# lh3/minimap2

Hardware: AMD Instinct MI355X
Metric: aligned Gbases/sec (map-ont, 10 kb reads, -a) (higher is better)
Workload: dtype int8 (ksw2 difference DP) / int32+f32 (chaining)

## Files before the change

minimap2_amd/__init__.py:

```python
import ctypes as C
import os

_HERE = os.path.dirname(os.path.abspath(__file__))
LIB_PATH = os.path.join(_HERE, "libmm2amd.so")


class Mm2AmdError(RuntimeError):
    pass


class KswJob(C.Structure):
    _fields_ = [("query", C.c_void_p), ("target", C.c_void_p), ("qlen", C.c_int32), ("tlen", C.c_int32), ("w", C.c_int32),
                ("zdrop", C.c_int32), ("end_bonus", C.c_int32), ("flag", C.c_int32)]


class FinJob(C.Structure):
    _fields_ = [("query", C.c_void_p), ("target", C.c_void_p), ("qlen", C.c_int32), ("tlen", C.c_int32), ("n_pieces", C.c_int32),
                ("piece", C.POINTER(C.POINTER(C.c_uint32))), ("piece_len", C.POINTER(C.c_int32))]


class FinRes(C.Structure):
    _fields_ = [("n_cigar", C.c_int32), ("blen", C.c_int32), ("mlen", C.c_int32), ("n_ambi", C.c_int32), ("dp_max", C.c_int32), ("qshift", C.c_int32),
                ("tshift", C.c_int32), ("is_spliced", C.c_int32), ("cigar_off", C.c_uint32)]

# ... 1197 lines not shown
        rc = lib().mm2amd_idx_getseq(self._idx, rid, start, end, buf)
        if rc < 0:
            _check(rc)
        return buf.raw.translate(_CODE_TO_BASE).decode("ascii")

    def map_pairs(self, pairs, text=False, cs=False, MD=False, ds=False):
        self.stage(pairs)
        if not text:
            return self.run(cs=cs, MD=MD, ds=ds)
        n_reg, reg, rep_len = self.run(raw=True)
        try:
            return self.format_raw(n_reg, reg, rep_len)
        finally:
            self.free_raw(n_reg, reg)

    def last_stats(self):
        v = (C.c_double * 48)()
        k = lib().mm2amd_last_stats(v, 48)
        names = ["t_seed_chain", "t_host_pre", "t_plan", "t_ksw", "t_consume", "t_finish", "n_jobs", "n_rounds", "dp_cells", "dev_allocs", "pin_allocs",
                 "alloc_ns", "cpu_seed_chain", "cpu_host_pre", "cpu_plan", "cpu_ksw", "cpu_consume", "cpu_finish", "n_long_join_dev", "n_long_join_host",
                 "drv_cpu_seed_chain", "drv_cpu_host_pre", "drv_cpu_plan", "drv_cpu_ksw", "drv_cpu_consume", "drv_cpu_finish", "n_early_sub",
                 "n_region_reads_dev", "n_region_reads_host", "n_band128", "n_band256", "n_band_widened", "n_band_rectangle",
                 "arena_dev_bytes", "arena_pin_bytes", "arena_dev_used", "arena_pin_used", "n_band512", "n_band_rectangle_big",
                 "n_anchors_prune_in", "n_anchors_prune_kept", "n_reads_prune_redo"]
        return dict(zip(names, list(v)[:k]))


class SplitWriter(object):

    def __init__(self, prefix, aligner, part_no):
        self._al, self._h = aligner, None
        self._h = lib().mm2amd_split_open(os.fsencode(prefix), aligner._idx, part_no)
        if not self._h:
            _check(lib().mm2amd_last_error_code())

    def write(self, n_seq, n_reg, reg, rep_len, frag_gap):
        _check(lib().mm2amd_split_write(self._h, C.byref(self._al.map_opt), n_seq, n_reg, reg, rep_len, frag_gap))

    def close(self):
        if self._h:
            h, self._h = self._h, None
            _check(lib().mm2amd_split_close(h))

    def __del__(self):
        try:
            self.close()
        except Exception:
# ... 140 lines not shown
```

minimap2_amd/csrc/backend_hip.cpp:

```cpp
#include <atomic>
#include <condition_variable>
#include <algorithm>
#include <cstdio>
#include <cstring>
#include <memory>
#include <mutex>
#include <numeric>
#include <stdexcept>
#include <thread>
#include "backend.hpp"
#include "chain_dump.hpp"
#include "chain_host.hpp"
#include "device_ctx.hpp"
#include "ksw_host.hpp"
#include "seed_chain_dev.hpp"
#include "index_build.hpp"
#include "kernel_prof.hpp"
#include "threads.hpp"
#include "trace.hpp"
#include "sdust_core.hpp"
#include "sdust.hpp"

namespace mm2amd {

extern const uint8_t kNt4Table[256];

namespace {

bool env_on(const char *name) { const char *e = getenv(name); return e && *e && strcmp(e, "0") != 0; }

struct Lane {
	int id = 0;
	int set = 0;
	hipStream_t stream = nullptr;
	SeedChainBuffers B{};
	KswRunner ksw;
	DevBuf<uint64_t> d_a_off, d_mp_off, d_mz_x, d_mz_y, d_minipos, d_skey_in, d_sval_in, d_skey_out, d_sval_out;
	DevBuf<uint32_t> d_sdust_list;
	DevBuf<SdustCounters> d_sdust_cnt;
	PinBuf<SdustCounters> h_sdust_cnt;
	DevBuf<uint32_t> d_mz_cnt, d_sd_n, d_sd_off, d_sd_aoff, d_sd_qpos, d_sd_info, d_n_anchor, d_n_minipos, d_n_seedhit, d_tie, d_nkept;
	DevBuf<int32_t> d_rep_len, d_f, d_p, d_t;
	DevBuf<Anchor> d_anchors;
	DevBuf<uint8_t> d_tbytes;
	DevBuf<uint32_t> d_sort_list;
	PinBuf<uint32_t> h_sort_list;
	DevBuf<Anchor> d_dump_anchors;
	DevBuf<uint32_t> d_pieces;
	PinBuf<uint32_t> h_pieces, h_lj_pieces;
	DevBuf<Anchor> d_lj_out_a;
	DevBuf<uint64_t> d_lj_src;
	PinBuf<Anchor> h_lj_a;
	PinBuf<uint64_t> h_lj_u, h_lj_off, h_lj_aoff, h_lj_uoff;
	PinBuf<int32_t> h_lj_nu, h_lj_nv;
	PinBuf<uint32_t> h_lj_tie, h_lj_list;
	PinBuf<unsigned long long> h_lj_cursor;
	DevBuf<FinRegion> d_fin_regions; DevBuf<FinPiece> d_fin_pieces; DevBuf<uint32_t> d_fin_out; DevBuf<FinResult> d_fin_res;
	PinBuf<FinRegion> h_fin_regions; PinBuf<FinPiece> h_fin_pieces; PinBuf<uint32_t> h_fin_out; PinBuf<FinResult> h_fin_res;
	struct EqxBufs { DevBuf<uint32_t> d_n, d_out; DevBuf<uint64_t> d_off; PinBuf<uint32_t> h_n, h_out; PinBuf<uint64_t> h_off; };
	EqxBufs eqx_fin, eqx_rg;
	long rg_lo = 0; size_t rg_n = 0; uint64_t rg_n_v = 0, rg_n_v2 = 0, rg_n_u = 0, rg_n_u2 = 0;
	std::vector<int8_t> rg_src; std::vector<uint64_t> rg_aoff, rg_uoff; std::vector<int32_t> rg_nu, rg_nv;
	DevBuf<uint64_t> d_lj_out_u;
// ... 124 lines not shown
			memcpy(h + seq_off_[i], reads[i].seq, reads[i].len);
			if (reads[i].paired()) memcpy(h + seq_off_[i] + reads[i].len, reads[i].seq2, reads[i].len2);
		}, 64);
		d_qpool_.ensure(2 * total + 16);
		d_seq_off_.ensure(n + 1);
		n_units_ = n;
		if (has_pairs_) {
			unit_first_.resize(n + 1);
			unit_first_[0] = 0;
			for (size_t i = 0; i < n; ++i) unit_first_[i + 1] = unit_first_[i] + (reads[i].paired() ? 2 : 1);
			n_units_ = (size_t)unit_first_[n];
			unit_off_.resize(n_units_ + 1);
			for (size_t i = 0; i < n; ++i) {
				unit_off_[unit_first_[i]] = seq_off_[i];
				if (reads[i].paired()) unit_off_[unit_first_[i] + 1] = seq_off_[i] + (uint64_t)reads[i].len;
			}
			unit_off_[n_units_] = total;
			d_unit_off_.ensure(n_units_ + 1), d_unit_first_.ensure(n + 1);
			HIP_CHECK(hipMemcpyAsync(d_unit_off_.p, unit_off_.data(), (n_units_ + 1) * 8, hipMemcpyHostToDevice, stream_));
			HIP_CHECK(hipMemcpyAsync(d_unit_first_.p, unit_first_.data(), (n + 1) * 4, hipMemcpyHostToDevice, stream_));
		}
		HIP_CHECK(hipMemcpyAsync(d_seq_off_.p, seq_off_.data(), (n + 1) * 8, hipMemcpyHostToDevice, stream_));
		read_names_.clear();
		if (getenv("MM2AMD_SEED_DUMP") || chain_dump_path()) for (size_t i = 0; i < n; ++i) read_names_.push_back(reads[i].name);
		have_read_names_ = false;
		if (name_rules_ && n > 0) {
			have_read_names_ = true;
			for (size_t i = 0; i < n; ++i) if (!reads[i].name) { have_read_names_ = false; break; }
		}
		if (have_read_names_) {
			name_key_.resize(2 * n);
			parallel_for_side(n_threads_, (long)n, [&](long i, int) {
				const std::string q(reads[i].name);
				const size_t lb = (size_t)(std::lower_bound(sorted_names_.begin(), sorted_names_.end(), q) - sorted_names_.begin());
				name_key_[i] = (int32_t)lb;
				name_key_[n + i] = lb < sorted_names_.size() && sorted_names_[lb] == q ? (int32_t)lb : -1;
			}, 256);
			d_name_key_.ensure(2 * n);
			HIP_CHECK(hipMemcpyAsync(d_name_key_.p, name_key_.data(), 2 * n * 4, hipMemcpyHostToDevice, stream_));
		}
		stream_wait(stream_);
	}
	void activate_batch() override { cur_ = 1 - cur_; }
	int current_set() const override { return cur_; }
	void bind_lane(int lane, int set) override { lanes_.at(lane)->set = set; }
	bool stages_beside_mapping() const override { return true; }

// ... 19 lines not shown
		B = SeedChainBuffers();
		B.n_reads = (int)n, B.seq_off = d_seq_off_.p + lo, B.ascii = h_ascii_.p, B.qpool = d_qpool_.p;
		if (have_read_names_) B.name_lb = d_name_key_.p + lo, B.name_eq = d_name_key_.p + seq_off_.size() - 1 + lo;
		KernelProfiler &kp = kernel_profiler(lane_id, replica_);
		double tt = Trace::now();
		const double L = (double)(seq_off_[hi] - seq_off_[lo]);
		SeedChainBuffers Bu = B;
		const size_t ulo = has_pairs_ ? (size_t)unit_first_[lo] : (size_t)lo, n_unit = has_pairs_ ? (size_t)unit_first_[hi] - ulo : n;
		if (has_pairs_) Bu.n_reads = (int)n_unit, Bu.seq_off = d_unit_off_.p + ulo;
		kp.begin(st); launch_encode(Bu, st); kp.end(st, "encode_kernel", 3 * L);
		const uint64_t base0 = seq_off_[lo], cap_mz = seq_off_[hi] - base0;
		ln.d_mz_cnt.ensure(n_unit);
		ln.d_mz_x.ensure(cap_mz + 1), ln.d_mz_y.ensure(cap_mz + 1);
		ln.d_sd_n.ensure(cap_mz + 1), ln.d_sd_off.ensure(cap_mz + 1), ln.d_sd_aoff.ensure(cap_mz + 1), ln.d_sd_qpos.ensure(cap_mz + 1), ln.d_sd_info.ensure(cap_mz + 1);
		B.mz_cnt = ln.d_mz_cnt.p, B.mz_off = B.seq_off, B.mz_x = ln.d_mz_x.p - base0, B.mz_y = ln.d_mz_y.p - base0;
		B.sd_n = ln.d_sd_n.p - base0, B.sd_off = ln.d_sd_off.p - base0, B.sd_aoff = ln.d_sd_aoff.p - base0, B.sd_qpos = ln.d_sd_qpos.p - base0, B.sd_info = ln.d_sd_info.p - base0;
		const double est_mz = 2.0 * L / (P.w + 1);
		Bu.mz_cnt = B.mz_cnt, Bu.mz_off = Bu.seq_off, Bu.mz_x = B.mz_x, Bu.mz_y = B.mz_y;
		int max_len = 0;
		for (size_t u = 0; u < n_unit; ++u) {
			const uint64_t l_u = has_pairs_ ? unit_off_[ulo + u + 1] - unit_off_[ulo + u] : seq_off_[lo + u + 1] - seq_off_[lo + u];
			max_len = (int)std::max<uint64_t>((uint64_t)max_len, l_u);
		}
		kp.begin(st); launch_sketch(Bu, P, max_len, st); kp.end(st, "sketch_kernel", L + 16.0 * est_mz);
		if (has_pairs_)
			B.unit_first = d_unit_first_.p + lo, B.unit_off = d_unit_off_.p, B.unit_cnt = ln.d_mz_cnt.p - ulo, B.mz_cnt = nullptr;
		const bool dev_sdust = P.sdust_thres > 0 && env_on("MM2AMD_DEVICE_SDUST"), sdust_no_narrow = env_on("MM2AMD_SDUST_NO_NARROW");
		if (dev_sdust) {
			ln.d_sdust_list.ensure(n_unit), ln.d_sdust_cnt.ensure(1);
			HIP_CHECK(hipMemsetAsync(ln.d_sdust_cnt.p, 0, sizeof(SdustCounters), st));
			SdustParams S;
			S.codes = B.qpool, S.off = Bu.seq_off, S.code_mul = 2, S.n_reads = (int)n_unit, S.T = P.sdust_thres < kSdustMaxT ? P.sdust_thres : kSdustMaxT;
			S.reg_n = B.sd_n, S.reg_s = B.sd_off, S.reg_e = B.sd_aoff, S.wide_list = ln.d_sdust_list.p, S.cnt = ln.d_sdust_cnt.p;
			const char *e_cap = getenv("MM2AMD_SDUST_NARROW_CAP");
			const long cap = e_cap && *e_cap ? strtol(e_cap, nullptr, 10) : kSdustNarrowCap;
			if (sdust_no_narrow) {
				S.cap = kSdustWideCap, S.wide = 2;
				kp.begin(st); sdust_launch(S, 0, st); kp.end(st, "sdust_kernel[wide]", 0.0);
			} else {
				S.cap = (int)(cap < 1 ? 1 : cap > kSdustWideCap ? kSdustWideCap : cap), S.wide = 0;
				kp.begin(st); sdust_launch(S, 0, st); kp.end(st, "sdust_kernel[narrow]", 0.0);
				S.cap = kSdustWideCap, S.wide = 1;
				kp.begin(st); sdust_launch(S, 0, st); kp.end(st, "sdust_kernel[wide]", 0.0);
			}
			HIP_CHECK(hipMemcpyAsync(ln.h_sdust_cnt.ensure(1), ln.d_sdust_cnt.p, sizeof(SdustCounters), hipMemcpyDeviceToHost, st));
			kp.begin(st); launch_dust_filter(B, st); kp.end(st, "dust_filter_kernel", 16.0 * est_mz);
		} else if (P.sdust_thres > 0) {
// ... 6 lines not shown
				thread_local std::vector<uint8_t> codes;
				codes.resize((size_t)len + 1);
				for (int j = 0; j < len; ++j) codes[j] = kNt4Table[(uint8_t)asc[o + j]];
				SdustState S;
				S.P = perf.data();
				uint32_t k = 0;
				sdust_scan(codes.data(), len, P.sdust_thres, S, [&](int s0, int e0) { h_s[o - base0 + k] = (uint32_t)s0, h_e[o - base0 + k] = (uint32_t)e0; ++k; });
				if (len > 0) h_n[o - base0] = k;
			}, 16);
			HIP_CHECK(hipMemcpyAsync(ln.d_sd_n.p, h_n, cap_mz * 4, hipMemcpyHostToDevice, st));
			HIP_CHECK(hipMemcpyAsync(ln.d_sd_off.p, h_s, cap_mz * 4, hipMemcpyHostToDevice, st));
			HIP_CHECK(hipMemcpyAsync(ln.d_sd_aoff.p, h_e, cap_mz * 4, hipMemcpyHostToDevice, st));
			kp.begin(st); launch_dust_filter(B, st); kp.end(st, "dust_filter_kernel", 16.0 * est_mz);
		}
		ln.d_n_anchor.ensure(n), ln.d_n_minipos.ensure(n), ln.d_n_seedhit.ensure(n), ln.d_rep_len.ensure(n);
		B.n_anchor = ln.d_n_anchor.p, B.n_minipos = ln.d_n_minipos.p, B.n_seedhit = ln.d_n_seedhit.p, B.rep_len = ln.d_rep_len.p;
		kp.begin(st); launch_seed_collect(B, I_, P, st); kp.end(st, "seed_collect_kernel", 36.0 * est_mz);
		uint32_t *h_na = ln.h_na.ensure(n), *h_nmp = ln.h_nmp.ensure(n);
		int32_t *h_rep = ln.h_rep.ensure(n);
		HIP_CHECK(hipMemcpyAsync(h_na, ln.d_n_anchor.p, n * 4, hipMemcpyDeviceToHost, st));
		HIP_CHECK(hipMemcpyAsync(h_nmp, ln.d_n_minipos.p, n * 4, hipMemcpyDeviceToHost, st));
		HIP_CHECK(hipMemcpyAsync(h_rep, ln.d_rep_len.p, n * 4, hipMemcpyDeviceToHost, st));
		stream_wait(st);
		if (dev_sdust) {
			const SdustCounters &c = *ln.h_sdust_cnt.p;
			if (c.err) throw HipError("[mm2amd] sdust_kernel: a list of perfect intervals outgrew the wide capacity");
			kp.add_units("sdust_kernel[wide]", (double)c.wide_bases);
			if (!sdust_no_narrow) kp.add_units("sdust_kernel[narrow]", L - (double)c.wide_bases + (double)c.narrow_partial);
		}
		Trace::get().add(lane_id, "gpu:sketch+collect", tt, Trace::now()); tt = Trace::now();
		std::vector<uint64_t> &a_off = ln.a_off, &mp_off = ln.mp_off;
		a_off.resize(n + 1), mp_off.resize(n + 1);
		a_off[0] = mp_off[0] = 0;
		for (size_t i = 0; i < n; ++i) a_off[i + 1] = a_off[i] + h_na[i], mp_off[i + 1] = mp_off[i] + h_nmp[i];
		const uint64_t n_a = a_off[n], n_mp = mp_off[n];
		uint64_t *h_off = ln.h_off.ensure(2 * (n + 1));
		memcpy(h_off, a_off.data(), (n + 1) * 8), memcpy(h_off + n + 1, mp_off.data(), (n + 1) * 8);
		ln.d_a_off.ensure(n + 1), ln.d_mp_off.ensure(n + 1);
		HIP_CHECK(hipMemcpyAsync(ln.d_a_off.p, h_off, (n + 1) * 8, hipMemcpyHostToDevice, st));
		HIP_CHECK(hipMemcpyAsync(ln.d_mp_off.p, h_off + n + 1, (n + 1) * 8, hipMemcpyHostToDevice, st));
		ln.d_anchors.ensure(n_a + 1), ln.d_minipos.ensure(n_mp + 1), ln.d_f.ensure(n_a + 1), ln.d_p.ensure(n_a + 1), ln.d_t.ensure(n_a + 1);
		ln.d_skey_in.ensure(n_a + 1), ln.d_sval_in.ensure(n_a + 1), ln.d_skey_out.ensure(n_a + 1), ln.d_sval_out.ensure(n_a + 1), ln.d_tie.ensure(2 * n + 1);
		B.sort_key_in = ln.d_skey_in.p, B.sort_val_in = ln.d_sval_in.p, B.sort_key_out = ln.d_skey_out.p, B.sort_val_out = ln.d_sval_out.p, B.tie_flag = ln.d_tie.p;
		B.tie_list = ln.d_tie.p + n, B.tie_count = ln.d_tie.p + 2 * n;
		B.rid_bits = rid_bits_;
		static const bool prune_env = !(getenv("MM2AMD_ANCHOR_PRUNE") && atoi(getenv("MM2AMD_ANCHOR_PRUNE")) == 0);
// ... 787 lines not shown
```

minimap2_amd/csrc/capi_kernels.cpp:

```cpp
#include <mutex>
#include <string>
#include <vector>
#include <cstring>
#include "../../include/mm2amd.h"
#include "hip_util.hpp"
#include "device_ctx.hpp"
#include "ksw_host.hpp"
#include "kernel_prof.hpp"
#include "region_finish.hpp"
#include "cigar_eqx.hpp"
#include "aln_text.hpp"
#include "junc_text.hpp"
#include "ksw_ll.hpp"
#include "sdust.hpp"
#include "sdust_core.hpp"
#include "hits_merge.hpp"
#include "split_merge.hpp"
#include "index_handle.hpp"
#include "fastx.hpp"
#include "threads.hpp"
#include "trace.hpp"
#include "device_sort.hpp"
#include "seed_chain_dev.hpp"
#include <map>
// ... 1087 lines not shown
			if (l) memcpy(h + o, seqs[i], l);
			o += l;
		}
		d_pool.ensure(2 * total + 32, 1.0), d_off.ensure(n_units + 1, 1.0);
		HIP_CHECK(hipMemsetAsync(d_pool.p, 0xff, 2 * total + 32, dc.stream));
		HIP_CHECK(hipMemcpyAsync(d_off.p, unit_off.data(), (n_units + 1) * 8, hipMemcpyHostToDevice, dc.stream));
		SeedChainBuffers B;
		B.n_reads = (int)(frag_unit[hi] - frag_unit[lo]), B.seq_off = d_off.p + frag_unit[lo], B.ascii = h, B.qpool = d_pool.p + 16;
		launch_encode(B, dc.stream);
		HIP_CHECK(hipMemcpyAsync(out, d_pool.p, 2 * total + 32, hipMemcpyDeviceToHost, dc.stream));
		HIP_CHECK(hipStreamSynchronize(dc.stream));
		return 0;
	});
}

long long mm2amd_alloc_counter(int which)
{
	AllocStats &a = alloc_stats();
	BandCounters &b = band_counters();
	return which == 0 ? a.dev_allocs.load() : which == 1 ? a.pin_allocs.load() : which == 2 ? a.ns.load() : which == 3 ? (long long)b.n_band1.load() : which == 4 ? (long long)b.n_band2.load() :
	       which == 5 ? (long long)b.n_widened.load() : which == 6 ? (long long)b.n_retried.load() :
	       which == 7 ? (long long)dev_arena().held_bytes() : which == 8 ? (long long)pin_arena().held_bytes() : which == 9 ? (long long)dev_arena().used_bytes() : which == 10 ? (long long)pin_arena().used_bytes() :
	       which == 11 ? (long long)b.n_band4.load() : which == 12 ? (long long)b.n_retried_big.load() :
	       which == 13 ? (long long)prune_counters().n_in.load() : which == 14 ? (long long)prune_counters().n_kept.load() : (long long)prune_counters().n_redo.load();
}

void mm2amd_profile_enable(int on)
{
	for (int r = 0; r < kMaxReplicas; ++r) for (int l = 0; l < kMaxProfLanes; ++l) kernel_profiler(l, r).reset();
	KernelProfiler::enabled_flag() = on != 0;
}

int mm2amd_profile_get(mm2amd_kernel_stat_t *out, int cap)
{
	std::map<std::string, KernelStat> all;
	for (int r = 0; r < kMaxReplicas; ++r) for (int l = 0; l < kMaxProfLanes; ++l)
		for (const auto &kv : kernel_profiler(l, r).stats()) {
			KernelStat &k = all[kv.first];
			k.ms += kv.second.ms, k.alg_bytes += kv.second.alg_bytes, k.units += kv.second.units, k.launches += kv.second.launches;
		}
	int n = 0;
	for (const auto &kv : all) {
		if (n >= cap) break;
		mm2amd_kernel_stat_t &o = out[n++];
		memset(&o, 0, sizeof o);
		strncpy(o.name, kv.first.c_str(), sizeof o.name - 1);
		o.ms = kv.second.ms, o.alg_bytes = kv.second.alg_bytes, o.launches = kv.second.launches, o.units = kv.second.units;
// ... 6 lines not shown
```

minimap2_amd/csrc/capi_map.cpp:

```cpp
#include <algorithm>
#include <condition_variable>
#include <cstdlib>
#include <cstring>
#include <memory>
#include <atomic>
#include <mutex>
#include <shared_mutex>
#include <string>
#include <thread>
#include "../../include/mm2amd.h"
#include "mapper.hpp"
#include "format.hpp"
#include "index_handle.hpp"
#include "threads.hpp"

namespace mm2amd {
int effective_cpus();
Backend *make_backend(const FlatIndex &fi, void *device_tables, int n_threads, int device, int replica, int tables_device);
int backend_device_count();
void *backend_build_index_tables(FlatIndex &fi, int device, int *on_device);
void backend_free_index_tables(void *tables);
const char *backend_name();
void capi_set_error(const std::string &msg);
int capi_fail(int code, const std::string &msg);
// ... 668 lines not shown
	std::unique_lock<std::shared_mutex> lk(g_ctx_mu);
	if (!g_ctx || g_ctx->generation != generation) return 0;
	g_ctx.reset();
	return 1;
}

const char *mm2amd_backend_name(void) { return backend_name(); }
int mm2amd_format_fraction(double v, char *buf) { return buf ? format_fraction_for_test(v, buf) : 0; }

int mm2amd_last_stats(double *v, int n)
{
	std::shared_lock<std::shared_mutex> lk(g_ctx_mu);
	if (!g_ctx) return 0;
	std::lock_guard<std::mutex> lk_stats(g_ctx->stats_mu);
	const MapperStats &s = g_ctx->stats;
	const double a[] = { s.t_seed_chain, s.t_host_pre, s.t_plan, s.t_ksw, s.t_consume, s.t_finish, (double)s.n_jobs, (double)s.n_rounds, s.dp_cells,
	                     (double)mm2amd_alloc_counter(0), (double)mm2amd_alloc_counter(1), (double)mm2amd_alloc_counter(2),
	                     s.c_seed_chain, s.c_host_pre, s.c_plan, s.c_ksw, s.c_consume, s.c_finish, (double)s.n_long_join_dev, (double)s.n_long_join_host,
	                     s.d_seed_chain, s.d_host_pre, s.d_plan, s.d_ksw, s.d_consume, s.d_finish, (double)s.n_early_sub,
	                     (double)s.n_region_reads_dev, (double)s.n_region_reads_host,
	                     (double)mm2amd_alloc_counter(3), (double)mm2amd_alloc_counter(4), (double)mm2amd_alloc_counter(5), (double)mm2amd_alloc_counter(6),
	                     (double)mm2amd_alloc_counter(7), (double)mm2amd_alloc_counter(8), (double)mm2amd_alloc_counter(9), (double)mm2amd_alloc_counter(10),
	                     (double)mm2amd_alloc_counter(11), (double)mm2amd_alloc_counter(12),
	                     (double)mm2amd_alloc_counter(13), (double)mm2amd_alloc_counter(14), (double)mm2amd_alloc_counter(15) };
	int k = 0;
	for (; k < n && k < (int)(sizeof a / sizeof a[0]); ++k) v[k] = a[k];
	return k;
}

}
```

minimap2_amd/csrc/hip_util.hpp:

```cpp
#pragma once
#include <hip/hip_runtime.h>
#include <time.h>
#include <cstdio>
#include <cstdlib>
#include <cstdint>
#include <stdexcept>
#include <string>
#include <atomic>
#include <chrono>
#include <map>
#include <mutex>
#include <vector>
#include <iterator>

#ifdef MM2AMD_WAVE_EMU
#define MM2_DYN_LDS(T, name) T *const name = (T *)wave_emu::dyn_shared()
#define MM2_LOCKSTEP() __builtin_amdgcn_wave_barrier()
#else
#define MM2_DYN_LDS(T, name) extern __shared__ __attribute__((aligned(16))) T name[]
#define MM2_LOCKSTEP() ((void)0)
#endif

namespace mm2amd {

// ... 27 lines not shown
	}
	HIP_CHECK(hipEventRecord(slot->ev, s));
	static const long max_ns = [] { const char *e = getenv("MM2AMD_WAIT_MAX_US"); const long us = e ? atol(e) : 500; return (us < 20 ? 20 : us) * 1000L; }();
	long ns = 20000;
	for (int it = 0;; ++it) {
		const hipError_t e = hipEventQuery(slot->ev);
		if (e == hipSuccess) return;
		if (e != hipErrorNotReady) HIP_CHECK(e);
		if (it < 4) continue;
		timespec ts = { 0, ns };
		nanosleep(&ts, nullptr);
		if (ns < max_ns) ns += ns / 2;
	}
}

int effective_cpus();

struct AllocStats { std::atomic<long> dev_allocs{0}, pin_allocs{0}; std::atomic<double> dummy{0}; std::atomic<long long> dev_bytes{0}, pin_bytes{0}; std::atomic<long long> ns{0}; };
inline AllocStats &alloc_stats() { static AllocStats s; return s; }
struct BandCounters { std::atomic<unsigned long long> n_band1{0}, n_band2{0}, n_band4{0}, n_widened{0}, n_retried{0}, n_retried_big{0}; };
inline BandCounters &band_counters() { static BandCounters s; return s; }
struct PruneCounters { std::atomic<unsigned long long> n_in{0}, n_kept{0}, n_redo{0}; };
inline PruneCounters &prune_counters() { static PruneCounters s; return s; }

class MemArena {
public:
	MemArena(bool pinned, size_t chunk_bytes) : pinned_(pinned), chunk_bytes_(chunk_bytes) {}
	~MemArena() { for (Chunk &c : chunks_) raw_free(c.base); for (auto &kv : solo_) raw_free(kv.first); }
	static bool enabled()
	{
#ifdef MM2AMD_WAVE_EMU
		static const bool on = getenv("MM2AMD_ARENA") != nullptr;
#else
		static const bool on = getenv("MM2AMD_NO_ARENA") == nullptr;
#endif
		return on;
	}
	void *alloc(size_t bytes)
	{
		bytes = (bytes + 255) & ~(size_t)255;
		if (bytes == 0) bytes = 256;
		int dev = 0;
		(void)hipGetDevice(&dev);
		if (!enabled() || bytes > chunk_bytes_ / 2) {
			char *p = raw_alloc(bytes);
			std::lock_guard<std::mutex> lk(mu_);
// ... 129 lines not shown
```

minimap2_amd/csrc/seed_chain.hip:

```cpp
#include <hip/hip_runtime.h>
#include "hip_util.hpp"
#include "seed_chain_dev.hpp"
#include "index_build.hpp"
#include "heap_order.hpp"
#include "sdust_core.hpp"
#include "sketch_dev.hpp"
#include "sdust_dev.hpp"
#include "kernel_prof.hpp"

namespace mm2amd {

#define WAVE_SYNC() do { __builtin_amdgcn_fence(__ATOMIC_ACQ_REL, "wavefront"); __builtin_amdgcn_wave_barrier(); } while (0)

__constant__ uint8_t c_nt4[256];
extern const uint8_t kNt4Table[256];
static bool g_nt4_uploaded = false;

static void upload_tables(hipStream_t s)
{
	if (g_nt4_uploaded) return;
	HIP_CHECK(hipMemcpyToSymbolAsync(HIP_SYMBOL(c_nt4), kNt4Table, 256, 0, hipMemcpyHostToDevice, s));
	g_nt4_uploaded = true;
}

constexpr int kEncodeBlocks = 64, kEncodeDepth = 4;

__device__ __forceinline__ int encode_owner(const uint64_t *seq_off, int lo, int n, uint64_t p)
{
	int step = 1;
// ... 129 lines not shown
	}
	if (min_x != UINT64_MAX) EMIT_MZ(min_x, min_y);
#undef EMIT_MZ
	B.mz_cnt[r] = n_out;
}

__device__ __forceinline__ uint32_t wave_prefix_add_u32(uint32_t v);
struct SketchLds {
	int ring_bytes, pk_words, tile_cap, per_wave;
};
__host__ __device__ inline SketchLds sketch_lds_layout(int w, int tile_cap)
{
	SketchLds L;
	L.tile_cap = tile_cap;
	L.ring_bytes = 64 * w * 12;
	if (L.ring_bytes < 1024) L.ring_bytes = 1024;
	L.pk_words = (tile_cap + 256) / 16;
	L.per_wave = L.ring_bytes + (L.pk_words + 2) * 4 + L.pk_words * 2 + tile_cap / 8;
	L.per_wave = (L.per_wave + 15) & ~15;
	return L;
}
constexpr int SK_WARM_LDS = 128, SK_TAIL_LDS = 128;

template <bool K32, int W>
__global__ void __launch_bounds__(64) sketch_wave_kernel(SeedChainBuffers B, int w, int k, int tile_cap)
{
	MM2_DYN_LDS(uint64_t, lds);
	const int lane = threadIdx.x;
	const int r = blockIdx.x;
	const SketchLds L = sketch_lds_layout(w, tile_cap);
	uint64_t *const bx = lds + lane;
	uint32_t *const by = (uint32_t *)(lds + (size_t)w * 64) + lane;
	uint32_t *const pk = (uint32_t *)((uint8_t *)lds + L.ring_bytes) + 2;
	uint16_t *const amb = (uint16_t *)(pk + L.pk_words);
	uint32_t *const marks = (uint32_t *)(amb + L.pk_words);
	uint16_t *const list = (uint16_t *)lds;
	const int list_cap = L.ring_bytes / 2;
	const uint64_t o = B.seq_off[r];
	const int64_t len = (int64_t)(B.seq_off[r + 1] - o);
	const uint8_t *seq = B.qpool + 2 * o;
	uint64_t *const ox = B.mz_x + B.mz_off[r], *const oy = B.mz_y + B.mz_off[r];
	if (lane == 0) pk[-1] = pk[-2] = 0;
	const int64_t n_tiles = len > tile_cap ? (len + tile_cap - 1) / tile_cap : 1;
	const int64_t tile = n_tiles > 1 ? ((len + n_tiles - 1) / n_tiles + 63) & ~(int64_t)63 : len;
	uint32_t n_out = 0;
	for (int64_t t0 = 0; t0 < len; t0 += tile) {
		const int64_t t1 = t0 + tile < len ? t0 + tile : len;
		const int64_t lo = t0 >= SK_WARM_LDS ? t0 - SK_WARM_LDS : 0;
		const int64_t hi = t1 + SK_TAIL_LDS < len ? t1 + SK_TAIL_LDS : len;
		for (int64_t c = lo + 16 * lane; c < hi; c += 16 * 64) {
			struct __attribute__((packed, aligned(1))) Q16 { uint32_t v[4]; };
			const Q16 q = *(const Q16 *)(seq + c);
			const uint32_t qv[4] = { q.v[0], q.v[1], q.v[2], q.v[3] };
			uint32_t packed, flags;
			sk_pack16(qv, &packed, &flags);
			pk[(c - lo) >> 4] = packed, amb[(c - lo) >> 4] = (uint16_t)flags;
		}
		for (int64_t i = lane; i < (t1 - t0 + 31) >> 5; i += 64) marks[i] = 0;
		WAVE_SYNC();
		int64_t chunk = (t1 - t0 + 63) / 64;
		if (chunk < 32) chunk = 32;
		const int64_t cs = t0 + (int64_t)lane * chunk, ce = cs + chunk < t1 ? cs + chunk : t1;
		if (cs < t1) {
			uint32_t wpk = 0, wamb = 0;
			int64_t wcur = -1;
			auto base_at = [&](int64_t i) -> int {
				if (i >= lo && i < hi) {
					const int64_t rel = i - lo;
					if ((rel >> 4) != wcur) wcur = rel >> 4, wpk = pk[wcur], wamb = amb[wcur];
					return (wamb >> (rel & 15) & 1u) ? 4 : (int)(wpk >> (30 - 2 * (int)(rel & 15)) & 3u);
				}
				return (int)seq[i];
			};
			sketch_chunk_core<false, K32, uint32_t, W>(base_at, len, cs, ce, w, k, 0u, bx, by, 64, [&](uint64_t, uint64_t y) {
				const uint32_t rel = (uint32_t)((int64_t)((uint32_t)y >> 1) - t0);
				atomicOr(&marks[rel >> 5], 1u << (rel & 31));
			}, (int64_t)(w + k + 8));
		}
		WAVE_SYNC();
		const int n_words = (int)((t1 - t0 + 31) >> 5);
		int words_per_round = list_cap / 32;
		if (words_per_round > 64) words_per_round = 64;
		for (int w0 = 0; w0 < n_words; w0 += words_per_round) {
			uint32_t m = lane < words_per_round && w0 + lane < n_words ? marks[w0 + lane] : 0u;
			const uint32_t cnt = (uint32_t)__popc(m);
			const uint32_t incl = wave_prefix_add_u32(cnt);
			const uint32_t total = (uint32_t)__builtin_amdgcn_readlane((int32_t)incl, 63);
			uint32_t at = incl - cnt;
			while (m) {
				list[at++] = (uint16_t)(((w0 + lane) << 5) + __builtin_ctz(m));
				m &= m - 1;
			}
			WAVE_SYNC();
			for (uint32_t e = lane; e < total; e += 64) {
				const int64_t pos = t0 + (int64_t)list[e];
				uint64_t x, y;
				sk_minimizer_at(pk, pos - lo, pos, k, &x, &y);
				ox[n_out + e] = x, oy[n_out + e] = y;
			}
			n_out += total;
			WAVE_SYNC();
		}
	}
	if (lane == 0) B.mz_cnt[r] = n_out;
}

void launch_sketch(const SeedChainBuffers &B, const SeedChainParams &P, int max_len, void *stream)
{
	hipStream_t s = (hipStream_t)stream;
	if (!P.is_hpc && P.w <= 32) {
		int tile_cap = (std::max(max_len, 1024) + 1023) & ~1023;
		if (tile_cap > 16384) tile_cap = 16384;
		static const int force_tile = getenv("MM2AMD_SKETCH_TILE") ? atoi(getenv("MM2AMD_SKETCH_TILE")) : 0;
		if (force_tile >= 64) tile_cap = force_tile & ~63;
		const SketchLds L = sketch_lds_layout(P.w, tile_cap);
#define MM2_SKETCH_LAUNCH(K32_, W_) hipLaunchKernelGGL((sketch_wave_kernel<K32_, W_>), dim3(B.n_reads), dim3(64), (size_t)L.per_wave, s, B, P.w, P.k, tile_cap)
		static const bool generic_only = getenv("MM2AMD_SKETCH_GENERIC") != nullptr;
		const bool k32 = 2 * P.k <= 32;
		if (generic_only) { if (k32) MM2_SKETCH_LAUNCH(true, 0); else MM2_SKETCH_LAUNCH(false, 0); }
		else if (k32 && P.w == 10) MM2_SKETCH_LAUNCH(true, 10);
		else if (k32 && P.w == 5) MM2_SKETCH_LAUNCH(true, 5);
		else if (!k32 && P.w == 19) MM2_SKETCH_LAUNCH(false, 19);
		else if (!k32 && P.w == 10) MM2_SKETCH_LAUNCH(false, 10);
		else if (k32) MM2_SKETCH_LAUNCH(true, 0);
		else MM2_SKETCH_LAUNCH(false, 0);
#undef MM2_SKETCH_LAUNCH
	} else {
		const dim3 grid((B.n_reads + 63) / 64), block(64);
		if (P.w <= 32) hipLaunchKernelGGL((sketch_kernel<32>), grid, block, 0, s, B, P.w, P.k, P.is_hpc);
		else hipLaunchKernelGGL((sketch_kernel<256>), grid, block, 0, s, B, P.w, P.k, P.is_hpc);
	}
	HIP_CHECK(hipGetLastError());
}

__global__ void __launch_bounds__(64) dust_filter_kernel(SeedChainBuffers B)
{
	const int r = blockIdx.x * 64 + threadIdx.x;
	if (r >= B.n_reads) return;
	const int32_t u0 = B.unit_first ? B.unit_first[r] : 0, nu = B.unit_first ? B.unit_first[r + 1] - u0 : 1;
	for (int32_t k = 0; k < nu; ++k) {
		const uint64_t o = B.unit_first ? B.unit_off[u0 + k] : B.seq_off[r];
		uint32_t *cnt = B.unit_first ? const_cast<uint32_t *>(B.unit_cnt) + (u0 + k) : B.mz_cnt + r;
		const uint32_t *rs = B.sd_off + o, *re = B.sd_aoff + o;
		const int n_reg = (int)B.sd_n[o];
		if (n_reg == 0) continue;
		const int pos_off = B.unit_first ? (int)(o - B.unit_off[u0]) : 0;
		*cnt = (uint32_t)dust_filter_minimizers((int)*cnt, B.mz_x + o, B.mz_y + o, n_reg,
			[&](int u, int32_t *st, int32_t *en) { *st = (int32_t)rs[u], *en = (int32_t)re[u]; }, pos_off);
	}
}

void launch_dust_filter(const SeedChainBuffers &B, void *stream)
{
	hipLaunchKernelGGL(dust_filter_kernel, dim3((B.n_reads + 63) / 64), dim3(64), 0, (hipStream_t)stream, B);
	HIP_CHECK(hipGetLastError());
// ... 1950 lines not shown
```

minimap2_amd/csrc/seed_chain_dev.hpp:

```cpp
#pragma once
#include <cstdint>
#include <cstddef>
#include "types.hpp"
#include "backend.hpp"

namespace mm2amd {

struct DevIndex {
	const uint32_t *bucket_start;
	const uint64_t *keys;
	const uint32_t *val_off;
	const struct IdxSlot *slots;
	const struct IdxSlot *first;
	const uint64_t *pos;
	const uint32_t *S;
	int bucket_bits, key_shift;
	const int32_t *name_rank;
	const uint32_t *seq_len;
};

struct SeedChainBuffers {
	int n_reads;
	const uint64_t *seq_off;
	const char *ascii;
	uint8_t *qpool;
	const int32_t *name_lb, *name_eq;
	const int32_t *unit_first;
	const uint64_t *unit_off;
	const uint32_t *unit_cnt;
	uint32_t *mz_cnt;
	const uint64_t *mz_off;
	uint64_t *mz_x, *mz_y;
	uint32_t *sd_n, *sd_off, *sd_aoff, *sd_qpos, *sd_info;
	uint32_t *n_anchor, *n_minipos, *n_seedhit;
	int32_t *rep_len;
	const uint64_t *a_off;
	const uint64_t *mp_off;
	Anchor *anchors;
	uint64_t *sort_key_in, *sort_val_in;
	uint64_t *sort_key_out, *sort_val_out;
	uint32_t *tie_flag;
	uint32_t *tie_list, *tie_count;
	int rid_bits;
	uint32_t *n_kept = nullptr;
	uint32_t *redo_list = nullptr, *redo_count = nullptr;
	int prune_bins = 0, prune_cap = 0;
	uint64_t *mini_pos;
	int32_t *f, *p, *t;
	const uint32_t *pieces = nullptr;
	int n_pieces = 0, piece_len = 0;
	int rmq_rank_max = 256;
	int piece_dense = 0;
	unsigned long long *bt_cursor;
	Anchor *bt_out_a;
	uint64_t *bt_out_u;
// ... 22 lines not shown
```

Baseline: 3.806.

## Add windowed parallel minimizer sketch with dirty-block sequential fallback

Adds a sketch kernel variant in which each lane of the wave evaluates one position, computing its hash key in parallel into an LDS ring. Each position is then tested directly for being a window minimizer by comparing it with its W neighbours. Only 64-position blocks that contain ties, ambiguous bases or nearby edges are recomputed with the existing sequential per-chunk core. This is intended to replace the mostly serial per-lane chunk scan, and its duplicated warm-up work, with data-parallel evaluation. It becomes the default for common w/k pairs and adds block/dirty counters, a per-call device-to-host copy, and extra LDS usage that could reduce occupancy.

```diff
diff --git a/minimap2_amd/__init__.py b/minimap2_amd/__init__.py
--- a/minimap2_amd/__init__.py
+++ b/minimap2_amd/__init__.py
@@ -1243,7 +1243,8 @@
                  "drv_cpu_seed_chain", "drv_cpu_host_pre", "drv_cpu_plan", "drv_cpu_ksw", "drv_cpu_consume", "drv_cpu_finish", "n_early_sub",
                  "n_region_reads_dev", "n_region_reads_host", "n_band128", "n_band256", "n_band_widened", "n_band_rectangle",
                  "arena_dev_bytes", "arena_pin_bytes", "arena_dev_used", "arena_pin_used", "n_band512", "n_band_rectangle_big",
-                 "n_anchors_prune_in", "n_anchors_prune_kept", "n_reads_prune_redo"]
+                 "n_anchors_prune_in", "n_anchors_prune_kept", "n_reads_prune_redo",
+                 "n_sketch_blocks", "n_sketch_blocks_dirty"]
         return dict(zip(names, list(v)[:k]))
 
 
diff --git a/minimap2_amd/csrc/backend_hip.cpp b/minimap2_amd/csrc/backend_hip.cpp
--- a/minimap2_amd/csrc/backend_hip.cpp
+++ b/minimap2_amd/csrc/backend_hip.cpp
@@ -39,6 +39,8 @@
 	DevBuf<uint32_t> d_sdust_list;
 	DevBuf<SdustCounters> d_sdust_cnt;
 	PinBuf<SdustCounters> h_sdust_cnt;
+	DevBuf<unsigned long long> d_sk_count; PinBuf<unsigned long long> h_sk_count; unsigned long long sk_seen[2] = { 0, 0 };
+	DevBuf<uint32_t> d_sk_blocks; PinBuf<uint32_t> h_sk_blocks;
 	DevBuf<uint32_t> d_mz_cnt, d_sd_n, d_sd_off, d_sd_aoff, d_sd_qpos, d_sd_info, d_n_anchor, d_n_minipos, d_n_seedhit, d_tie, d_nkept;
 	DevBuf<int32_t> d_rep_len, d_f, d_p, d_t;
 	DevBuf<Anchor> d_anchors;
@@ -209,7 +211,7 @@
 		}
 		HIP_CHECK(hipMemcpyAsync(d_seq_off_.p, seq_off_.data(), (n + 1) * 8, hipMemcpyHostToDevice, stream_));
 		read_names_.clear();
-		if (getenv("MM2AMD_SEED_DUMP") || chain_dump_path()) for (size_t i = 0; i < n; ++i) read_names_.push_back(reads[i].name);
+		if (getenv("MM2AMD_SEED_DUMP") || getenv("MM2AMD_SKETCH_TRACE") || chain_dump_path()) for (size_t i = 0; i < n; ++i) read_names_.push_back(reads[i].name);
 		have_read_names_ = false;
 		if (name_rules_ && n > 0) {
 			have_read_names_ = true;
@@ -275,7 +277,15 @@
 			const uint64_t l_u = has_pairs_ ? unit_off_[ulo + u + 1] - unit_off_[ulo + u] : seq_off_[lo + u + 1] - seq_off_[lo + u];
 			max_len = (int)std::max<uint64_t>((uint64_t)max_len, l_u);
 		}
+		static const bool sk_trace = getenv("MM2AMD_SKETCH_TRACE") != nullptr;
+		if (!ln.d_sk_count.p) { ln.d_sk_count.ensure(2); HIP_CHECK(hipMemsetAsync(ln.d_sk_count.p, 0, 16, st)); }
+		Bu.sk_count = ln.d_sk_count.p;
+		if (sk_trace) Bu.sk_blocks = ln.d_sk_blocks.ensure(2 * n_unit);
 		kp.begin(st); launch_sketch(Bu, P, max_len, st); kp.end(st, "sketch_kernel", L + 16.0 * est_mz);
+		unsigned long long *h_skc = ln.h_sk_count.ensure(2);
+		HIP_CHECK(hipMemcpyAsync(h_skc, ln.d_sk_count.p, 16, hipMemcpyDeviceToHost, st));
+		uint32_t *h_skb = sk_trace ? ln.h_sk_blocks.ensure(2 * n_unit) : nullptr;
+		if (sk_trace) HIP_CHECK(hipMemcpyAsync(h_skb, ln.d_sk_blocks.p, 2 * n_unit * 4, hipMemcpyDeviceToHost, st));
 		if (has_pairs_)
 			B.unit_first = d_unit_first_.p + lo, B.unit_off = d_unit_off_.p, B.unit_cnt = ln.d_mz_cnt.p - ulo, B.mz_cnt = nullptr;
 		const bool dev_sdust = P.sdust_thres > 0 && env_on("MM2AMD_DEVICE_SDUST"), sdust_no_narrow = env_on("MM2AMD_SDUST_NO_NARROW");
@@ -328,6 +338,19 @@
 		HIP_CHECK(hipMemcpyAsync(h_nmp, ln.d_n_minipos.p, n * 4, hipMemcpyDeviceToHost, st));
 		HIP_CHECK(hipMemcpyAsync(h_rep, ln.d_rep_len.p, n * 4, hipMemcpyDeviceToHost, st));
 		stream_wait(st);
+		{
+			sketch_counters().n_blocks += h_skc[0] - ln.sk_seen[0], sketch_counters().n_dirty += h_skc[1] - ln.sk_seen[1];
+			ln.sk_seen[0] = h_skc[0], ln.sk_seen[1] = h_skc[1];
+			if (sk_trace && !has_pairs_) {
+				std::string txt;
+				char buf[64];
+				for (size_t i = 0; i < n; ++i) {
+					txt += "[mm2amd] SKETCH read ", txt += read_names_.empty() || !read_names_[lo + i] ? "*" : read_names_[lo + i];
+					snprintf(buf, sizeof buf, ": blocks %u dirty %u\n", h_skb[2 * i], h_skb[2 * i + 1]), txt += buf;
+				}
+				fputs(txt.c_str(), stderr);
+			}
+		}
 		if (dev_sdust) {
 			const SdustCounters &c = *ln.h_sdust_cnt.p;
 			if (c.err) throw HipError("[mm2amd] sdust_kernel: a list of perfect intervals outgrew the wide capacity");
diff --git a/minimap2_amd/csrc/capi_kernels.cpp b/minimap2_amd/csrc/capi_kernels.cpp
--- a/minimap2_amd/csrc/capi_kernels.cpp
+++ b/minimap2_amd/csrc/capi_kernels.cpp
@@ -1133,7 +1133,8 @@
 	       which == 5 ? (long long)b.n_widened.load() : which == 6 ? (long long)b.n_retried.load() :
 	       which == 7 ? (long long)dev_arena().held_bytes() : which == 8 ? (long long)pin_arena().held_bytes() : which == 9 ? (long long)dev_arena().used_bytes() : which == 10 ? (long long)pin_arena().used_bytes() :
 	       which == 11 ? (long long)b.n_band4.load() : which == 12 ? (long long)b.n_retried_big.load() :
-	       which == 13 ? (long long)prune_counters().n_in.load() : which == 14 ? (long long)prune_counters().n_kept.load() : (long long)prune_counters().n_redo.load();
+	       which == 13 ? (long long)prune_counters().n_in.load() : which == 14 ? (long long)prune_counters().n_kept.load() : which == 15 ? (long long)prune_counters().n_redo.load() :
+	       which == 16 ? (long long)sketch_counters().n_blocks.load() : (long long)sketch_counters().n_dirty.load();
 }
 
 void mm2amd_profile_enable(int on)
diff --git a/minimap2_amd/csrc/capi_map.cpp b/minimap2_amd/csrc/capi_map.cpp
--- a/minimap2_amd/csrc/capi_map.cpp
+++ b/minimap2_amd/csrc/capi_map.cpp
@@ -714,7 +714,8 @@
 	                     (double)mm2amd_alloc_counter(3), (double)mm2amd_alloc_counter(4), (double)mm2amd_alloc_counter(5), (double)mm2amd_alloc_counter(6),
 	                     (double)mm2amd_alloc_counter(7), (double)mm2amd_alloc_counter(8), (double)mm2amd_alloc_counter(9), (double)mm2amd_alloc_counter(10),
 	                     (double)mm2amd_alloc_counter(11), (double)mm2amd_alloc_counter(12),
-	                     (double)mm2amd_alloc_counter(13), (double)mm2amd_alloc_counter(14), (double)mm2amd_alloc_counter(15) };
+	                     (double)mm2amd_alloc_counter(13), (double)mm2amd_alloc_counter(14), (double)mm2amd_alloc_counter(15),
+	                     (double)mm2amd_alloc_counter(16), (double)mm2amd_alloc_counter(17) };
 	int k = 0;
 	for (; k < n && k < (int)(sizeof a / sizeof a[0]); ++k) v[k] = a[k];
 	return k;
diff --git a/minimap2_amd/csrc/hip_util.hpp b/minimap2_amd/csrc/hip_util.hpp
--- a/minimap2_amd/csrc/hip_util.hpp
+++ b/minimap2_amd/csrc/hip_util.hpp
@@ -73,6 +73,8 @@
 inline BandCounters &band_counters() { static BandCounters s; return s; }
 struct PruneCounters { std::atomic<unsigned long long> n_in{0}, n_kept{0}, n_redo{0}; };
 inline PruneCounters &prune_counters() { static PruneCounters s; return s; }
+struct SketchCounters { std::atomic<unsigned long long> n_blocks{0}, n_dirty{0}; };
+inline SketchCounters &sketch_counters() { static SketchCounters s; return s; }
 
 class MemArena {
 public:
diff --git a/minimap2_amd/csrc/seed_chain.hip b/minimap2_amd/csrc/seed_chain.hip
--- a/minimap2_amd/csrc/seed_chain.hip
+++ b/minimap2_amd/csrc/seed_chain.hip
@@ -5,6 +5,7 @@
 #include "heap_order.hpp"
 #include "sdust_core.hpp"
 #include "sketch_dev.hpp"
+#include "sketch_window_dev.hpp"
 #include "sdust_dev.hpp"
 #include "kernel_prof.hpp"
 
@@ -180,20 +181,26 @@
 }
 constexpr int SK_WARM_LDS = 128, SK_TAIL_LDS = 128;
 
-template <bool K32, int W>
+template <bool K32, int W, bool WIN = false>
 __global__ void __launch_bounds__(64) sketch_wave_kernel(SeedChainBuffers B, int w, int k, int tile_cap)
 {
 	MM2_DYN_LDS(uint64_t, lds);
+	typedef typename SkwKeyType<K32>::type KT;
 	const int lane = threadIdx.x;
 	const int r = blockIdx.x;
 	const SketchLds L = sketch_lds_layout(w, tile_cap);
+	const SkwLds LW = skw_lds_layout(w, tile_cap, (int)sizeof(KT));
+	const int ring_lanes = WIN ? skw_dirty_lanes(W, (int)sizeof(KT)) : 64, front_bytes = WIN ? LW.front_bytes : L.ring_bytes;
 	uint64_t *const bx = lds + lane;
-	uint32_t *const by = (uint32_t *)(lds + (size_t)w * 64) + lane;
-	uint32_t *const pk = (uint32_t *)((uint8_t *)lds + L.ring_bytes) + 2;
+	uint32_t *const by = (uint32_t *)(lds + (size_t)w * ring_lanes) + lane;
+	KT *const keys = (KT *)((uint8_t *)lds + LW.key_off);
+	uint16_t *const dlist = (uint16_t *)((uint8_t *)lds + LW.dlist_off);
+	uint32_t *const pk = (uint32_t *)((uint8_t *)lds + front_bytes) + 2;
 	uint16_t *const amb = (uint16_t *)(pk + L.pk_words);
 	uint32_t *const marks = (uint32_t *)(amb + L.pk_words);
 	uint16_t *const list = (uint16_t *)lds;
-	const int list_cap = L.ring_bytes / 2;
+	const int list_cap = front_bytes / 2;
+	uint32_t n_blocks = 0, n_dirty = 0;
 	const uint64_t o = B.seq_off[r];
 	const int64_t len = (int64_t)(B.seq_off[r + 1] - o);
 	const uint8_t *seq = B.qpool + 2 * o;
@@ -214,26 +221,74 @@
 			sk_pack16(qv, &packed, &flags);
 			pk[(c - lo) >> 4] = packed, amb[(c - lo) >> 4] = (uint16_t)flags;
 		}
-		for (int64_t i = lane; i < (t1 - t0 + 31) >> 5; i += 64) marks[i] = 0;
+		if (!WIN) for (int64_t i = lane; i < (t1 - t0 + 31) >> 5; i += 64) marks[i] = 0;
 		WAVE_SYNC();
-		int64_t chunk = (t1 - t0 + 63) / 64;
-		if (chunk < 32) chunk = 32;
-		const int64_t cs = t0 + (int64_t)lane * chunk, ce = cs + chunk < t1 ? cs + chunk : t1;
-		if (cs < t1) {
-			uint32_t wpk = 0, wamb = 0;
-			int64_t wcur = -1;
-			auto base_at = [&](int64_t i) -> int {
-				if (i >= lo && i < hi) {
-					const int64_t rel = i - lo;
-					if ((rel >> 4) != wcur) wcur = rel >> 4, wpk = pk[wcur], wamb = amb[wcur];
-					return (wamb >> (rel & 15) & 1u) ? 4 : (int)(wpk >> (30 - 2 * (int)(rel & 15)) & 3u);
-				}
-				return (int)seq[i];
-			};
-			sketch_chunk_core<false, K32, uint32_t, W>(base_at, len, cs, ce, w, k, 0u, bx, by, 64, [&](uint64_t, uint64_t y) {
-				const uint32_t rel = (uint32_t)((int64_t)((uint32_t)y >> 1) - t0);
-				atomicOr(&marks[rel >> 5], 1u << (rel & 31));
-			}, (int64_t)(w + k + 8));
+		uint32_t wpk = 0, wamb = 0;
+		int64_t wcur = -1;
+		auto base_at = [&](int64_t i) -> int {
+			if (i >= lo && i < hi) {
+				const int64_t rel = i - lo;
+				if ((rel >> 4) != wcur) wcur = rel >> 4, wpk = pk[wcur], wamb = amb[wcur];
+				return (wamb >> (rel & 15) & 1u) ? 4 : (int)(wpk >> (30 - 2 * (int)(rel & 15)) & 3u);
+			}
+			return (int)seq[i];
+		};
+		if constexpr (WIN) {
+			const int nb = (int)((t1 - t0 + 63) >> 6), margin = skw_margin(W, k);
+			const bool tiny = len - (k - 1) < W || t1 - t0 < W;
+			uint64_t bad_a = 0, bad_b = 0, nm_prev = 0;
+			int nd = 0;
+			for (int i = -2; i <= nb + 1; ++i) {
+				const int q = 64 * i + lane, pos = (int)t0 + q;
+				const uint64_t nm = __ballot(skw_is_n(amb, pos, (int)lo, (int)hi));
+				KT key = skw_key_at<K32>(pk, pos, (int)lo, (int)hi, k);
+				if (nm | nm_prev) {
+					if (skw_n_spread(nm_prev, nm, k) >> lane & 1) key = 0;
+				}
+				keys[q & 255] = key, keys[(q & 255) + 256] = key;
+				WAVE_SYNC();
+				uint64_t bad_c = 0;
+				if (i >= 0) {
+					const int b = i - 1, x0 = (64 * b) & 255;
+					bool mark, tie;
+					skw_lane_eval<KT, W>(keys + (x0 ? x0 : 256) + lane, &mark, &tie);
+					bad_c = __ballot(tie) | nm_prev;
+					const uint64_t mk = __ballot(mark && pos - 64 >= (int)t0 && pos - 64 < (int)t1);
+					if (b >= 0 && b < nb && lane < 2) marks[2 * b + lane] = (uint32_t)(mk >> (32 * lane));
+				}
+				if (i >= 2 && (tiny || skw_block_dirty(bad_a, bad_b, bad_c, margin))) {
+					if (lane == 0) dlist[nd] = (uint16_t)(i - 2);
+					++nd;
+				}
+				bad_a = bad_b, bad_b = bad_c, nm_prev = nm;
+			}
+			WAVE_SYNC();
+			n_blocks += (uint32_t)nb, n_dirty += (uint32_t)nd;
+			const int quota = skw_dirty_quota(nd, ring_lanes);
+			if (lane < ring_lanes && lane * quota < nd) {
+				const int e1 = (lane + 1) * quota < nd ? (lane + 1) * quota : nd;
+				for (int e = lane * quota; e < e1;) {
+					int f = e + 1;
+					while (f < e1 && dlist[f] == dlist[f - 1] + 1) ++f;
+					const int b0 = dlist[e], b1 = dlist[f - 1] + 1;
+					for (int b = b0; b < b1; ++b) marks[2 * b] = marks[2 * b + 1] = 0;
+					const int64_t cs = t0 + 64 * (int64_t)b0, ce = t0 + 64 * (int64_t)b1 < t1 ? t0 + 64 * (int64_t)b1 : t1;
+					sketch_chunk_core<false, K32, uint32_t, W>(base_at, len, cs, ce, w, k, 0u, bx, by, ring_lanes, [&](uint64_t, uint64_t y) {
+						const uint32_t rel = (uint32_t)((int64_t)((uint32_t)y >> 1) - t0);
+						marks[rel >> 5] |= 1u << (rel & 31);
+					}, (int64_t)margin);
+					e = f;
+				}
+			}
+		} else {
+			int64_t chunk = (t1 - t0 + 63) / 64;
+			if (chunk < 32) chunk = 32;
+			const int64_t cs = t0 + (int64_t)lane * chunk, ce = cs + chunk < t1 ? cs + chunk : t1;
+			if (cs < t1)
+				sketch_chunk_core<false, K32, uint32_t, W>(base_at, len, cs, ce, w, k, 0u, bx, by, 64, [&](uint64_t, uint64_t y) {
+					const uint32_t rel = (uint32_t)((int64_t)((uint32_t)y >> 1) - t0);
+					atomicOr(&marks[rel >> 5], 1u << (rel & 31));
+				}, (int64_t)(w + k + 8));
 		}
 		WAVE_SYNC();
 		const int n_words = (int)((t1 - t0 + 31) >> 5);
@@ -261,20 +316,39 @@
 		}
 	}
 	if (lane == 0) B.mz_cnt[r] = n_out;
+	if (WIN && lane == 0) {
+		if (B.sk_count) {
+			atomicAdd(&B.sk_count[0], (unsigned long long)n_blocks);
+			if (n_dirty) atomicAdd(&B.sk_count[1], (unsigned long long)n_dirty);
+		}
+		if (B.sk_blocks) B.sk_blocks[2 * r] = n_blocks, B.sk_blocks[2 * r + 1] = n_dirty;
+	}
 }
 
 void launch_sketch(const SeedChainBuffers &B, const SeedChainParams &P, int max_len, void *stream)
 {
 	hipStream_t s = (hipStream_t)stream;
+	bool win = false;
 	if (!P.is_hpc && P.w <= 32) {
 		int tile_cap = (std::max(max_len, 1024) + 1023) & ~1023;
 		if (tile_cap > 16384) tile_cap = 16384;
 		static const int force_tile = getenv("MM2AMD_SKETCH_TILE") ? atoi(getenv("MM2AMD_SKETCH_TILE")) : 0;
 		if (force_tile >= 64) tile_cap = force_tile & ~63;
 		const SketchLds L = sketch_lds_layout(P.w, tile_cap);
+		static const bool window_on = !getenv("MM2AMD_SKETCH_WINDOW") || atoi(getenv("MM2AMD_SKETCH_WINDOW")) != 0;
 #define MM2_SKETCH_LAUNCH(K32_, W_) hipLaunchKernelGGL((sketch_wave_kernel<K32_, W_>), dim3(B.n_reads), dim3(64), (size_t)L.per_wave, s, B, P.w, P.k, tile_cap)
 		static const bool generic_only = getenv("MM2AMD_SKETCH_GENERIC") != nullptr;
 		const bool k32 = 2 * P.k <= 32;
+		win = window_on && !generic_only && skw_supported(P.w, P.k) && (k32 ? P.w == 10 || P.w == 5 : P.w == 19 || P.w == 10);
+		const SkwLds LW = skw_lds_layout(P.w, tile_cap, k32 ? 4 : 8);
+#define MM2_SKETCH_LAUNCH_WIN(K32_, W_) hipLaunchKernelGGL((sketch_wave_kernel<K32_, W_, true>), dim3(B.n_reads), dim3(64), (size_t)LW.per_wave, s, B, P.w, P.k, tile_cap)
+		if (win) {
+			if (k32 && P.w == 10) MM2_SKETCH_LAUNCH_WIN(true, 10);
+			else if (k32) MM2_SKETCH_LAUNCH_WIN(true, 5);
+			else if (P.w == 19) MM2_SKETCH_LAUNCH_WIN(false, 19);
+			else MM2_SKETCH_LAUNCH_WIN(false, 10);
+		} else
+#undef MM2_SKETCH_LAUNCH_WIN
 		if (generic_only) { if (k32) MM2_SKETCH_LAUNCH(true, 0); else MM2_SKETCH_LAUNCH(false, 0); }
 		else if (k32 && P.w == 10) MM2_SKETCH_LAUNCH(true, 10);
 		else if (k32 && P.w == 5) MM2_SKETCH_LAUNCH(true, 5);
@@ -289,6 +363,7 @@
 		else hipLaunchKernelGGL((sketch_kernel<256>), grid, block, 0, s, B, P.w, P.k, P.is_hpc);
 	}
 	HIP_CHECK(hipGetLastError());
+	if (B.sk_blocks && !win) HIP_CHECK(hipMemsetAsync(B.sk_blocks, 0, (size_t)B.n_reads * 8, s));
 }
 
 __global__ void __launch_bounds__(64) dust_filter_kernel(SeedChainBuffers B)
diff --git a/minimap2_amd/csrc/seed_chain_dev.hpp b/minimap2_amd/csrc/seed_chain_dev.hpp
--- a/minimap2_amd/csrc/seed_chain_dev.hpp
+++ b/minimap2_amd/csrc/seed_chain_dev.hpp
@@ -31,6 +31,8 @@
 	uint32_t *mz_cnt;
 	const uint64_t *mz_off;
 	uint64_t *mz_x, *mz_y;
+	unsigned long long *sk_count = nullptr;
+	uint32_t *sk_blocks = nullptr;
 	uint32_t *sd_n, *sd_off, *sd_aoff, *sd_qpos, *sd_info;
 	uint32_t *n_anchor, *n_minipos, *n_seedhit;
 	int32_t *rep_len;
diff --git a/minimap2_amd/csrc/sketch_window_dev.hpp b/minimap2_amd/csrc/sketch_window_dev.hpp
--- /dev/null
+++ b/minimap2_amd/csrc/sketch_window_dev.hpp
@@ -0,0 +1,125 @@
+#pragma once
+#include <hip/hip_runtime.h>
+#include <cstdint>
+#include "sketch_dev.hpp"
+
+namespace mm2amd {
+
+template <bool K32> struct SkwKeyType { typedef uint64_t type; };
+template <> struct SkwKeyType<true> { typedef uint32_t type; };
+
+__host__ __device__ inline int skw_margin(int w, int k) { return w + k + 8; }
+__host__ __device__ inline bool skw_supported(int w, int k) { return (k & 1) && w >= 2 && skw_margin(w, k) <= 63 && skw_margin(w, k) + w <= 65; }
+__host__ __device__ inline int skw_dirty_lanes(int w, int key_bytes) { return 32 * w * 12 + 512 * key_bytes + 1024 <= 64 * w * 12 ? 32 : 16; }
+
+template <bool K32>
+__device__ __forceinline__ typename SkwKeyType<K32>::type skw_key_at(const uint32_t *pk, int pos, int lo, int hi, int k)
+{
+	typedef typename SkwKeyType<K32>::type KT;
+	if (pos < lo + k - 1 || pos >= hi) return 0;
+	const int r = pos - lo, j = r >> 4;
+	if (K32) {
+		const uint32_t mask = (1u << 2 * k) - 1u;
+		const uint32_t k0 = (uint32_t)(((uint64_t)pk[j - 1] << 32 | pk[j]) >> (30 - 2 * (r & 15))) & mask;
+#if defined(__has_builtin) && __has_builtin(__builtin_bitreverse32)
+		uint32_t y = __builtin_bitreverse32(k0);
+		y = (y >> 1 & 0x55555555u) | (y & 0x55555555u) << 1;
+		const uint32_t k1 = (y >> (32 - 2 * k)) ^ mask;
+#else
+		const uint32_t k1 = (uint32_t)sk_revcomp(k0, k);
+#endif
+		return (KT)(mm_hash_t<uint32_t>(k0 < k1 ? k0 : k1, mask) + 1u);
+	}
+	const uint64_t mask = (1ULL << 2 * k) - 1ULL;
+	const uint64_t k0 = sk_kmer_at(pk, r, k), k1 = sk_revcomp(k0, k);
+	return (KT)(mm_hash_t<uint64_t>(k0 < k1 ? k0 : k1, mask) + 1ULL);
+}
+__device__ __forceinline__ bool skw_is_n(const uint16_t *amb, int pos, int lo, int hi)
+{
+	return pos >= lo && pos < hi && (amb[(pos - lo) >> 4] >> ((pos - lo) & 15) & 1);
+}
+__host__ __device__ inline uint64_t skw_n_spread(uint64_t prev, uint64_t cur, int k)
+{
+	uint64_t lo = prev, hi = cur;
+	int have = 1;
+	while (have < k) {
+		const int sh = have * 2 <= k ? have : k - have;
+		hi |= hi << sh | lo >> (64 - sh), lo |= lo << sh;
+		have += sh;
+	}
+	return hi;
+}
+
+template <typename KT, int W>
+__device__ __forceinline__ void skw_lane_eval(const KT *c, bool *mark, bool *tie)
+{
+	const KT x = c[0];
+	if (sizeof(KT) == 4) {
+		uint32_t rmin[W], lmin = UINT32_MAX, t = UINT32_MAX;
+		rmin[0] = UINT32_MAX;
+#pragma unroll
+		for (int d = 1; d < W; ++d) {
+			const uint32_t r = (uint32_t)c[d];
+			rmin[d] = rmin[d - 1] < r ? rmin[d - 1] : r;
+			t = t < (r ^ (uint32_t)x) ? t : r ^ (uint32_t)x;
+		}
+		uint32_t best = rmin[W - 1];
+#pragma unroll
+		for (int d = 1; d < W; ++d) {
+			const uint32_t l = (uint32_t)c[-d];
+			lmin = lmin < l ? lmin : l;
+			t = t < (l ^ (uint32_t)x) ? t : l ^ (uint32_t)x;
+			const uint32_t both = lmin < rmin[W - 1 - d] ? lmin : rmin[W - 1 - d];
+			best = best > both ? best : both;
+		}
+		const uint32_t tl = (uint32_t)c[-W] ^ (uint32_t)x, tr = (uint32_t)c[W] ^ (uint32_t)x;
+		t = t < tl ? t : tl, t = t < tr ? t : tr;
+		*mark = (best > (uint32_t)x) & (x != 0), *tie = (t == 0) & (x != 0);
+		return;
+	}
+	bool lrun[W];
+	bool eq = false;
+	lrun[0] = true;
+#pragma unroll
+	for (int d = 1; d < W; ++d) {
+		const KT l = c[-d];
+		lrun[d] = lrun[d - 1] & (l > x);
+		eq |= l == x;
+	}
+	bool m = lrun[W - 1], rrun = true;
+#pragma unroll
+	for (int d = 1; d < W; ++d) {
+		const KT r = c[d];
+		rrun &= r > x;
+		eq |= r == x;
+		m |= lrun[W - 1 - d] & rrun;
+	}
+	eq |= (c[-W] == x) | (c[W] == x);
+	*mark = m & (x != 0), *tie = eq & (x != 0);
+}
+
+__host__ __device__ inline bool skw_block_dirty(uint64_t prev, uint64_t cur, uint64_t next, int margin)
+{
+	return cur != 0 || (margin > 0 && ((prev >> (64 - margin)) != 0 || (next & ((1ULL << margin) - 1ULL)) != 0));
+}
+__host__ __device__ inline int skw_dirty_quota(int nd, int lanes) { return (nd + lanes - 1) / lanes; }
+
+struct SkwLds {
+	int ring_bytes, key_off, dlist_off, front_bytes, pk_words, tile_cap, per_wave;
+};
+__host__ __device__ inline SkwLds skw_lds_layout(int w, int tile_cap, int key_bytes)
+{
+	SkwLds L;
+	L.tile_cap = tile_cap;
+	L.ring_bytes = skw_dirty_lanes(w, key_bytes) * w * 12;
+	L.key_off = L.ring_bytes;
+	L.dlist_off = L.key_off + 512 * key_bytes;
+	L.front_bytes = L.dlist_off + 2 * (tile_cap / 64 + 1);
+	L.front_bytes = (L.front_bytes + 15) & ~15;
+	L.pk_words = (tile_cap + 256) / 16;
+	L.per_wave = L.front_bytes + (L.pk_words + 2) * 4 + L.pk_words * 2 + tile_cap / 8;
+	L.per_wave = (L.per_wave + 15) & ~15;
+	return L;
+}
+
+}
```

Result: no change. 3.851, median of 6 (+1.2%).
